# Amelie-Schreiber/ShapeMol

Measured on AMD Instinct MI355X. Metric: molecules/sec (1000-step DDPM sample, batch 256), higher is better.
Workload: dtype f32 (matrix operands split exactly into 3 x bf16 pieces = 24 bits, six piece products, fp32 accumulate); 1 GPU; BASELINE configs[1]: batch 256 MOSES-prior molecules (9-27 atoms) per GPU, 1000-step chain, fp32 results, k=8, synthetic shapes + hash-filled weights; besides the 5 warm-up steps an untimed 200-step chain runs first to reach the loaded clocks; batch_per_gpu=256, atoms_per_gpu=5541, total_atoms=5541, noise=device Philox, trajectories=kept in HBM, launch=hipGraph replay, parallelism=dp1 (whole batches per rank), ranks_seen=1

## Files before the change

### shapemol_amd/csrc/probe_node_only.hip

```cpp
#include "../../include/shapemol_hip.h"
#include "sm_device.h"
#include "sm_edge.h"
#include "sm_edge_bf16.h"
#include "sm_edge16.h"
#include "sm_node.h"
template __global__ void node_chain6_kernel<128>(NodeChainArgs);
template __global__ void node_linear6_kernel<128>(NodeLinArgs);
template __global__ void node_prologue6_kernel<128>(NodePrologueArgs);
```

### shapemol_amd/csrc/shapemol_hip.hip

```cpp
#include "../../include/shapemol_hip.h"
#include "sm_device.h"
#include "sm_edge.h"
#include "sm_edge_bf16.h"
#include "sm_edge16.h"
#include "sm_node.h"
#include "sm_node16.h"
#include "sm_edge_stream.h"
#include "sm_misc.h"
#include "sm_cfg.h"
#include "sm_guide_groups.h"
#include "sm_mesh.h"
#include <hip/hip_ext.h>

#include <algorithm>
#include <cmath>
#include <type_traits>
#include <cstdio>
#include <cstring>
#include <map>
#include <string>
#include <vector>

#include "sm_pack.h"

// ... 62 lines not shown
    float *x_a = nullptr, *x_b = nullptr, *x_state = nullptr, *pred_pos = nullptr, *pred_v = nullptr;
    int64_t *v_state = nullptr;
    unsigned long long *stamps = nullptr;
    unsigned long long *kstamps = nullptr;
    int kstamp_sel = -1;
    int stamp_on = 0;
    double *bn_acc = nullptr;
    int *status = nullptr;
    ChainParams *chain_params = nullptr;
    int64_t lastN = 0, lastB = 0;
    const float *last_h = nullptr, *last_x = nullptr;
    int stop_layer = -1, edge_threads = 0 , lin_waves = 16, edge_bf16 = 2, lin_bf16 = 1, chain_bf16 = 1, vn_fuse = 2;
    int vn_fold = 1;
    int max_mol_atoms = 0;
    int stream_whole_rounds = 0;
    int lin_fuse = 0;
    int bn_eval = 0;
    float *bn_run = nullptr;
    double *bn_eval_acc = nullptr;
    int ddpm_fold = 1;
    DdpmFold ddpm_vf{};
    int graph_fuse = 1;
    int x2h_chain = 1;
    int node_f16 = 0;
    int feat_f16 = 0;
    int edge_tiles = -1;
    float hid_max = 0.f;
    int num_cu = 256;
    CloudSet cs; MeshSet ms;
    int2 *wg_table = nullptr; int64_t wg_table_cap = 0;
    shapemol_sd_ctx *field_sd = nullptr; double field_lr = 0.0; int field_step = 0;
    float4 *m_within = nullptr; int *m_out = nullptr, *m_cnt = nullptr; int64_t m_cap = 0, m_cnt_cap = 0;
    int64_t m_flag_groups = 0;
    double cfg_w = 0.0, cfg_p = 0.0; int cfg_type = 0, cfg_has_bounds = 0; float cfg_lo[3] = {}, cfg_hi[3] = {};
    float *cfg_tr_pos_u = nullptr, *cfg_tr_v_u = nullptr;
    float *inv_u = nullptr, *add0_u = nullptr, *addp_u = nullptr, *ps_u = nullptr, *pred_pos_u = nullptr, *pred_v_u = nullptr;
    float *shape_zero = nullptr;
    ShapeTermArgs *prep_terms_u = nullptr; VnShapeArgs *prep_vn_u = nullptr;
    float *cfg_stat = nullptr; double *cfg_part = nullptr; unsigned *cfg_hist = nullptr;
    CfgGroupSet cgs;
    int *cfg_mol_grp = nullptr; int2 *cfg_blk_tab = nullptr; double *cfg_gpart = nullptr; int64_t cfg_tab_stride = 0;
    int first_step = 0;
    int *pin_off = nullptr, *pin_atom = nullptr, *pin_nbr = nullptr; int64_t n_pins = 0; int pin_steps = 0, pin_k = 0;
    bool prof_on = false;
    std::vector<ProfRec> prof;
    hipEvent_t cur_e0 = nullptr, cur_e1 = nullptr;
    hipGraphExec_t gexec = nullptr, gexec_u = nullptr;
    int64_t n_captures = 0;
    int64_t launch_rec[8] = {}, graph_rec[8] = {};
    struct GraphKey { int64_t N = 0, B = 0; Guide guide = Guide::None; int fold = 0, gfuse = 0;
                      int cfg = 0 ; double cfgv[9] = {};
                      int cfg_groups = 0;
                      uint64_t field_gen = 0; double field_lr = 0.0; int field_step = 0;
                      bool operator==(const GraphKey &o) const {
                          if (!(N == o.N && B == o.B && guide == o.guide && fold == o.fold && gfuse == o.gfuse && cfg == o.cfg &&
                                cfg_groups == o.cfg_groups && field_gen == o.field_gen && field_lr == o.field_lr &&
                                field_step == o.field_step)) return false;
                          for (int i = 0; i < 9; ++i) if (cfgv[i] != o.cfgv[i]) return false;
                          return true;
                      } } gkey{};
    hipStream_t gstream = nullptr; bool gstream_set = false;
    void drop_graphs() {
        if (!gexec && !gexec_u) return;
        if (!gstream_set || hipStreamSynchronize(gstream) != hipSuccess) hipDeviceSynchronize();
        if (gexec) { hipGraphExecDestroy(gexec); gexec = nullptr; }
        if (gexec_u) { hipGraphExecDestroy(gexec_u); gexec_u = nullptr; }
    }
    const float *P(size_t off) const { return d_img + off; }
};

namespace {

// ... 115 lines not shown
    constexpr int vn_tail = vn_red_doubles(12, H / 8) * 8 + 12 * 96 * 4;
    constexpr int fold = K <= 16 ? kVnFoldBytes : 0;
    constexpr int x16 = 2 * EdgeImage16<H, NT>::TOTAL * 4 + fold, h16 = (EdgeImage16<H, NT>::TOTAL + EdgeImage16<H, 1>::TOTAL) * 4 + vn_tail;
    ATTR(x16, edge16_kernel<H, K, false>); ATTR(x16, edge16_kernel<H, K, false, true>);
    ATTR(x16, edge16_loop_kernel<H, K, false>); ATTR(x16, edge16_loop_kernel<H, K, false, true>);
    ATTR(h16, edge16_kernel<H, K, true>); ATTR(h16, edge16_kernel<H, K, true, true>);
    ATTR(h16, edge16_loop_kernel<H, K, true>); ATTR(h16, edge16_loop_kernel<H, K, true, true>);
    ATTR((StreamMap<H, false>::O_TAIL * 4 + kVnFoldBytes), edge_stream_kernel<H, K, false>);
    ATTR((StreamMap<H, true>::O_TAIL * 4 + (NT + kStreamProducers) * 64 * 2 * 8), edge_stream_kernel<H, K, true>);
    if constexpr (K <= 16) {
        constexpr int xph = EdgePhaseImage<H, NT>::TOTAL * 4, hph = (EdgePhaseImage<H, NT>::TOTAL + EdgePhaseImage<H, 1>::TOTAL) * 4 + vn_tail;
        ATTR(x16, x2h_chain16_kernel<H, K>); ATTR(x16, x2h_chain16_kernel<H, K, true>);
        ATTR((EdgeBlob<H, false>::TOTAL * 4), edge_attention_kernel<H, K, false>); ATTR((EdgeBlob<H, true>::TOTAL * 4), edge_attention_kernel<H, K, true>);
        ATTR(xph, edge_fused_kernel<H, K, false, false>); ATTR(xph, edge_fused_kernel<H, K, false, true>);
        ATTR(hph, edge_fused_kernel<H, K, true, false>); ATTR(hph, edge_fused_kernel<H, K, true, true>);
    }
    return 0;
}

template <int H>
int set_edge_attr(int KP) {
    constexpr size_t pro6 = 2 * Chain6Lds<H>::FRAG * 16 + Chain6Lds<H>::PRE * 4, pro16 = 2 * Chain16Lds<H>::FRAG * 16 + Chain16Lds<H>::PRE * 4;
    ATTR(pro6, node_prologue6_kernel<H>); ATTR(Chain6Lds<H>::BYTES, node_chain6_kernel<H>); ATTR(kLin6Chunk * 3 * H * 32, node_linear6_kernel<H>);
    ATTR(pro16, node_prologue16_kernel<H>); ATTR(Chain16Lds<H>::BYTES, node_chain16_kernel<H>); ATTR(kLin16Chunk * 2 * H * 32, node_linear16_kernel<H>);
    ATTR(pro16, node_prologue16_kernel<H, true>); ATTR(Chain16Lds<H>::BYTES, node_chain16_kernel<H, true>); ATTR(kLin16Chunk * 2 * H * 32, node_linear16_kernel<H, true>);
    return KP == 8 ? set_edge_attr_k<H, 8>() : (KP == 16 ? set_edge_attr_k<H, 16>() : set_edge_attr_k<H, 32>());
}
#undef ATTR

#define SM_ARGS(...) __VA_ARGS__
#define LAUNCH_KP(name, K, KERNEL, TAIL, ...) LAUNCH(name, SMK((KERNEL<H, K SM_ARGS TAIL>), __VA_ARGS__))
#define DISPATCH_KP16(name, KERNEL, TAIL, ...)                                                      \
    do { if (KP == 8) LAUNCH_KP(name, 8, KERNEL, TAIL, __VA_ARGS__); else LAUNCH_KP(name, 16, KERNEL, TAIL, __VA_ARGS__); } while (0)
#define DISPATCH_KP(name, KERNEL, TAIL, ...)                                                        \
    do { if (KP > 16) LAUNCH_KP(name, 32, KERNEL, TAIL, __VA_ARGS__); else DISPATCH_KP16(name, KERNEL, TAIL, __VA_ARGS__); } while (0)
#define DISPATCH_KP_F16(DISPATCH, name, KERNEL, TAIL, ...)                                          \
    do { if (c->feat_f16) DISPATCH(name, KERNEL, (SM_ARGS TAIL, true), __VA_ARGS__); else DISPATCH(name, KERNEL, TAIL, __VA_ARGS__); } while (0)

static int edge_waves_for(const shapemol_ctx *c, int njobs) {
    if (c->edge_threads > 0) return c->edge_threads / 64;
    return std::max(4, std::min(12, (njobs + c->num_cu - 1) / c->num_cu));
}

template <int H, bool H2X>
int launch_edge(shapemol_ctx *c, hipStream_t s, const EdgeArgs &a) {
    const int KP = c->KP;
// ... 129 lines not shown
template <int H>
int launch_linear(shapemol_ctx *c, hipStream_t s, const char *name, const float *in, const float *wimg, const float *wimg6, const float *wimg16, const float *add_mol,
                  int ld_add, float *out, int ld_out, int n_out_tiles, int n_atoms, unsigned long long *stamps) {
    const int nwave = c->lin_waves;
    const int n_ct = (n_atoms + 15) / 16, ogroups = (n_out_tiles + nwave - 1) / nwave;
    const int want_groups = std::max(1, c->num_cu / ogroups);
    const int tpg = std::max(1, (n_ct + want_groups - 1) / want_groups);
    const int agroups = (n_ct + tpg - 1) / tpg;
    const bool f16 = c->lin_bf16 && c->node_f16;
    NodeLinArgs a{in, f16 ? wimg16 : (c->lin_bf16 ? wimg6 : wimg), add_mol, c->mol_of, out, n_atoms, n_out_tiles, tpg, ld_add, ld_out, stamps, nwave};
    if (f16) {
        const size_t shm = (size_t)std::min(tpg, kLin16Chunk) * 2 * H * 32;
        if (c->feat_f16) LAUNCH(name, SMK((node_linear16_kernel<H, true>), dim3(ogroups * agroups), dim3(nwave * 64), shm, s, a, c->status + ST_RANGE));
        else LAUNCH(name, SMK(node_linear16_kernel<H>, dim3(ogroups * agroups), dim3(nwave * 64), shm, s, a, c->status + ST_RANGE));
    } else if (c->lin_bf16) {
        const size_t shm = (size_t)std::min(tpg, kLin6Chunk) * 3 * H * 32;
        LAUNCH(name, SMK(node_linear6_kernel<H>, dim3(ogroups * agroups), dim3(nwave * 64), shm, s, a));
    } else {
        LAUNCH(name, SMK(node_linear_kernel<H>, dim3(ogroups * agroups), dim3(nwave * 64), 0, s, a));
    }
    return 0;
}

NodeFollow follow_of(const shapemol_ctx *c, const DevMlpImg &m, int mode, float *out, int ld_out, int n_store) {
    NodeFollow f{};
    f.w1img = c->P(m.w1img); f.b1 = c->P(m.b1); f.ln_g = c->P(m.g); f.ln_b = c->P(m.be);
    f.w1img6 = c->P(c->node_f16 ? m.w1img16 : m.w1img6); f.w2img6 = c->P(c->node_f16 ? m.w2img16 : m.w2img6);
    f.w2img = c->P(m.w2img); f.b2 = c->P(m.b2); f.out = out; f.ld_out = ld_out; f.n_store = n_store; f.mode = mode; f.nt2 = m.nt2;
    return f;
}

__global__ void knn_pin_kernel(const int *off, int n_steps, const int *atom, const int *pnbr, int k, int kp, const int *step_cur, int n_atoms, int *nbr) {
    const int step = *step_cur;
    if (step < 0 || step >= n_steps) return;
    const int lo = off[step], hi = off[step + 1];
    for (int e = lo + blockIdx.x * blockDim.x + threadIdx.x; e < hi; e += gridDim.x * blockDim.x) {
        const int i = atom[e];
        if (i < 0 || i >= n_atoms) continue;
        for (int sl = 0; sl < kp; ++sl) nbr[(size_t)i * kp + sl] = sl < k ? pnbr[(size_t)e * k + sl] : -1;
    }
}

template <int H>
int run_prep_shape(shapemol_ctx *c, hipStream_t s, int64_t B, const float *d_shape);

void swap_uncond(shapemol_ctx *c) {
// ... 158 lines not shown
    const int L = g.num_layers, hd = g.n_heads, C = g.num_classes, D = g.time_emb_dim, KP = c->KP;
    const int n = (int)N;
    AtomEmbArgs ae{c->P(c->dm.embw), c->P(c->dm.embb), v_in, c->mol_of, c->ttab, c->t_mol, sampling ? c->steps : nullptr,
                   c->steps + 1, c->bn_acc, c->h_a, n, H, C, D, t_first, L * kBnReplicas * 2 * hd + L};
    const int nlay = c->stop_layer >= 0 ? std::min(c->stop_layer, L) : L;
    const bool fused_prologue = c->chain_bf16 && c->lin_bf16;
    if (fused_prologue && c->prologue_tab) {
        if (c->tab_key != prologue_tab_key(c)) return fail("run_score: the prologue tables are not built for this precision mode");
        PrologueTabArgs ta{c->etab, c->q_tab, c->pre_tab, c->tab_flag, v_in, c->mol_of, c->t_mol, ae.step_ptr, ae.step_cur, c->bn_acc,
                           c->add0, c->h_a, c->q_x, c->pre0, c->status + ST_RANGE, n, C, g.num_timesteps, t_first, ae.bn_acc_len};
        LAUNCH("node_prologue", SMK(node_prologue_tab_kernel<H>, dim3((unsigned)((N * 16 + kProTabThreads - 1) / kProTabThreads)), dim3(kProTabThreads), 0, s, ta));
    } else if (fused_prologue) {
        NodePrologueArgs pa = prologue_args<H>(c, v_in, c->mol_of, c->t_mol, c->add0, c->h_a, c->q_x, c->pre0, n);
        pa.step_ptr = ae.step_ptr; pa.step_cur = ae.step_cur; pa.bn_acc = c->bn_acc; pa.bn_acc_len = ae.bn_acc_len; pa.t_first = t_first;
        if (nlay == 0) pa.n_lin_tiles = 0;
        pa.stamps = c->kstamp_sel == 5 ? c->kstamps : nullptr;
        if (launch_prologue<H>(c, s, pa)) return 1;
    } else {
        LAUNCH("embed", SMK(atom_embed_kernel, dim3((N * H + 255) / 256), dim3(256), 0, s, ae));
    }
    const bool graph_fused = sampling && c->graph_fuse && c->max_mol_atoms > 0 && c->max_mol_atoms <= kGraphCap && KP <= 32 && c->n_pins == 0;
    int64_t (&rec)[8] = c->launch_rec;
    std::fill(rec, rec + 8, 0);
    rec[0] = sampling; rec[1] = graph_fused; rec[7] = c->num_cu;
    if (c->edge_bf16 == 2 && nlay > 0) { rec[5] = stream_chunk(c, n); rec[6] = (stream_jobs(c, n) + rec[5] - 1) / rec[5]; }
    if (reuse_graph) {
    } else if (graph_fused) {
        GraphArgs ga{x_in, c->mol_span, n, g.knn, KP, c->nbr, c->P(c->dm.ew.w1), c->P(c->dm.ew.b1), c->P(c->dm.ew.g), c->P(c->dm.ew.be),
                     c->P(c->dm.ew.w2), c->P(c->dm.ew.b2), c->ew, c->status + ST_SPAN, c->kstamp_sel == 4 ? c->kstamps : nullptr};
        const int apb = kGraphWaves * (KP >= 16 ? 1 : 16 / KP);
        DISPATCH_KP("graph", graph_kernel, (), dim3((n + apb - 1) / apb), dim3(kGraphWaves * 64), 0, s, ga);
    } else LAUNCH("knn", SMK(knn_kernel, dim3((N + 3) / 4), dim3(256), 0, s, x_in, c->mol_of, c->mol_off, n, g.knn, KP, c->nbr));
    if (sampling && c->n_pins > 0 && !reuse_graph)
        LAUNCH("knn", SMK(knn_pin_kernel, dim3(32), dim3(256), 0, s, c->pin_off, c->pin_steps, c->pin_atom, c->pin_nbr, c->pin_k, KP, c->steps + 1, n, c->nbr));
    EdgeWeightArgs ea{x_in, c->nbr, c->P(c->dm.ew.w1), c->P(c->dm.ew.b1), c->P(c->dm.ew.g), c->P(c->dm.ew.be),
                      c->P(c->dm.ew.w2), c->P(c->dm.ew.b2), c->ew, n * KP, KP};
    if (!graph_fused && !reuse_graph) {
        const int tiles = (n * KP + 15) / 16;
        LAUNCH("edge_weight", SMK(edge_weight_kernel<H>, dim3((tiles + 3) / 4), dim3(256), 0, s, ea));
    }
    const float *cur_x = x_in;
    float *cur_h = c->h_a;
    constexpr int NT = H / 16;
    bool v_done = false;
    if (nlay > 0 && !fused_prologue) {
        const DevLayer &D0 = c->dm.layer[0];
// ... 46 lines not shown
        } else {
            EdgeArgs e{c->P(Dl.blob_x2h), pre_x, c->q_x, cur_x, c->nbr, c->ew, c->att, n, ld_pre_x, stamps_x};
            if (launch_edge<H, false>(c, s, e)) return 1;
        }
        {
            float *dst = (last && out_h) ? out_h : (cur_h == c->h_a ? c->h_b : c->h_a);
            NodeChainArgs na{};
            na.att = c->att; na.h = cur_h; na.h_out = dst; na.n_atoms = n;
            na.stamps = (c->kstamp_sel == 3 && l == 0) ? c->kstamps : nullptr;
            na.w1img = c->P(Dl.no.w1img); na.b1 = c->P(Dl.no.b1); na.ln_g = c->P(Dl.no.g); na.ln_b = c->P(Dl.no.be);
            na.w2img = c->P(Dl.no.w2img); na.b2 = c->P(Dl.no.b2);
            na.w1img6 = c->P(c->node_f16 ? Dl.no.w1img16 : Dl.no.w1img6); na.w2img6 = c->P(c->node_f16 ? Dl.no.w2img16 : Dl.no.w2img6);
            na.f[0] = follow_of(c, Dl.q_h2x, NODE_LN_RELU, c->q_h, H, H);
            na.n_follow = 1;
            if (has_next) { na.f[1] = follow_of(c, c->dm.layer[l + 1].q_x2h, NODE_LN_RELU, c->q_x, H, H); na.n_follow = 2; }
            else if (out_v) { na.f[1] = follow_of(c, c->dm.vhead, NODE_SSP, out_v, C, C); na.n_follow = 2; v_done = true; }
            const int n_ct = (n + 15) / 16;
            const int lin_tiles = (has_next && l + 1 < L ? 8 : 4) * NT;
            const bool lin_fused = c->chain_bf16 && c->lin_bf16 && c->node_f16 && c->lin_fuse;
            if (lin_fused) {
                na.lin_img16 = c->P(Dl.lin16_img); na.add_mol = c->addp + (size_t)l * c->capB * 8 * H; na.mol_of = c->mol_of;
                na.pre_out = c->preAB; na.n_lin_tiles = lin_tiles; na.ld_add = 8 * H; na.ld_out = 8 * H;
            }
            if (xc_fused) { rec[4] = 1; if (launch_x2h_chain<H>(c, s, xea, na)) return 1; }
            else if (c->chain_bf16 && c->node_f16 && c->feat_f16) LAUNCH("node_chain", SMK((node_chain16_kernel<H, true>), dim3((n_ct + CHAIN_COLS - 1) / CHAIN_COLS), dim3(H * 4), Chain16Lds<H>::BYTES, s, na, c->status + ST_RANGE));
            else if (c->chain_bf16 && c->node_f16) LAUNCH("node_chain", SMK(node_chain16_kernel<H>, dim3((n_ct + CHAIN_COLS - 1) / CHAIN_COLS), dim3(H * 4), Chain16Lds<H>::BYTES, s, na, c->status + ST_RANGE));
            else if (c->chain_bf16) LAUNCH("node_chain", SMK(node_chain6_kernel<H>, dim3((n_ct + CHAIN_COLS - 1) / CHAIN_COLS), dim3(H * 4), Chain6Lds<H>::BYTES, s, na));
            else LAUNCH("node_chain", SMK(node_chain_kernel<H>, dim3((n_ct + CHAIN_COLS - 1) / CHAIN_COLS), dim3(H * 4), 0, s, na));
            cur_h = dst;
            if (!lin_fused && launch_linear<H>(c, s, "node_pre", cur_h, c->P(Dl.lin_img), c->P(Dl.lin6_img), c->P(Dl.lin16_img), c->addp + (size_t)l * c->capB * 8 * H, 8 * H,
                                 c->preAB, 8 * H, lin_tiles, n, (c->kstamp_sel == 0 && l == 0) ? c->kstamps : nullptr)) return 1;
        }
        float *x_next = (last && out_pos) ? out_pos : ((cur_x == c->x_a) ? c->x_b : c->x_a);
        bool vn_done = false, stats_done = false;
        unsigned long long *stamps_h = (c->kstamp_sel == 2 && l == 0) ? c->kstamps : nullptr;
        if ((f16 || stream) && c->vn_fuse != 1) {
            const H2xPlan plan = h2x_plan(c, l, fold, has_next, half_tiles, stat_acc, cur_x, x_next, out_pos);
            pending = plan.pending; stats_done = plan.stats_done; vn_done = plan.vn_done;
            if (plan.ddpm.enable) c->ddpm_vf = plan.ddpm;
            rec[2] |= plan.pending.enable; rec[3] |= plan.ddpm.enable;
            if (f16) {
                Edge16Args ea{};
                ea.image_k = c->P(Dl.i16_kh); ea.image_v = c->P(Dl.i16_vh);
                fill_edge(ea, c, c->preAB, 8 * H, c->q_h, cur_x, c->o3, n, half_tiles, stamps_h);
                ea.vn = plan.vn; ea.xsum = plan.xsum;
                if (launch_edge16<H, true>(c, s, ea)) return 1;
            } else {
                EdgeStreamArgs sa{};
                sa.part_k = c->P(Dl.st_kh); sa.part_v = c->P(Dl.st_vh);
                sa.w2k = reinterpret_cast<const unsigned *>(c->P(Dl.sw2_kh));
                fill_edge(sa, c, c->preAB, 8 * H, c->q_h, cur_x, c->o3, n, half_tiles, stamps_h);
                sa.vn = plan.vn; sa.xsum = plan.xsum;
                if (launch_stream<H, true>(c, s, sa)) return 1;
// ... 318 lines not shown
    else if (k == "edge_bf16") {
        if (value < 0 || value > 3) return fail("edge_bf16 must be 0 (fp32 MFMA), 1 (exactly split bf16, phase kernels), 2 (exactly split bf16, streaming kernels) or 3 (two-piece f16)");
        if (value != 3 && value != 2 && c->KP > 16) return fail("k > 16 runs on the streaming (edge_bf16 = 2) or the two-piece f16 (edge_bf16 = 3) edge kernels");
        if (value == 3 && c->hid_max > 6.0e4f) return fail("edge_bf16 = 3: the edge MLPs' LayerNorm outputs may exceed the fp16 range for these weights");
        c->edge_bf16 = (int)value;
    }
    else if (k == "edge_tiles") { if (value < -1 || value > 1) return fail("edge_tiles must be -1 (automatic), 0 (sliced one-job launches) or 1 (looping launch)"); c->edge_tiles = (int)value; }
    else if (k == "node_f16") c->node_f16 = value != 0;
    else if (k == "feat_f16") {
        if (value && (c->edge_bf16 != 3 || !c->node_f16)) return fail("feat_f16 = 1 needs the f16 kernels (edge_bf16 = 3, node_f16 = 1)");
        c->feat_f16 = value != 0;
    }
    else if (k == "lin_fuse") c->lin_fuse = value != 0;
    else if (k == "stream_whole_rounds") c->stream_whole_rounds = value != 0;
    else if (k == "x2h_chain") c->x2h_chain = value != 0;
    else if (k == "graph_fuse") c->graph_fuse = value != 0;
    else if (k == "bn_eval") c->bn_eval = value != 0;
    else if (k == "ddpm_fold") c->ddpm_fold = value != 0;
    else if (k == "vn_fold") c->vn_fold = value != 0;
    else if (k == "prologue_tab") c->prologue_tab = value != 0;
    else if (k == "lin_bf16") c->lin_bf16 = (int)value;
    else if (k == "chain_bf16") c->chain_bf16 = (int)value;
    else if (k == "vn_fuse") c->vn_fuse = (int)value;
    else if (k == "lin_waves") { if (value < 1 || value > 16) return fail("lin_waves must be 1..16"); c->lin_waves = (int)value; }
    else if (k == "stamps") c->stamp_on = (int)value;
    else if (k == "kstamp_sel") c->kstamp_sel = (int)value;
    else if (k == "edge_waves") { if (value < 0 || value > 12) return fail("edge_waves must be 0 (automatic) .. 12"); c->edge_threads = (int)value * 64; }
    else return fail("unknown option " + k);
    hipSetDevice(c->device);
    c->drop_graphs();
    return 0;
}

int64_t shapemol_debug_read(shapemol_ctx *c, const char *name, void *dst, size_t max_bytes) {
    if (!c || !name || !dst) { fail("shapemol_debug_read: null argument"); return -1; }
    const std::string k(name);
    const shapemol_config &g = c->cfg;
    const int64_t N = c->lastN;
    const void *src = nullptr; size_t bytes = 0;
    int64_t dims[8] = {N, c->lastB, c->KP, g.hidden_dim, g.n_heads, g.num_layers, c->capN, c->capB};
    if (k == "dims") { if (max_bytes < sizeof(dims)) return -1; std::memcpy(dst, dims, sizeof(dims)); return sizeof(dims); }
    if (k == "captures") { if (max_bytes < 8) return -1; std::memcpy(dst, &c->n_captures, 8); return 8; }
    if (k == "launch") { if (max_bytes < sizeof(c->launch_rec)) return -1; std::memcpy(dst, c->launch_rec, sizeof(c->launch_rec)); return sizeof(c->launch_rec); }
    if (k == "nbr") { src = c->nbr; bytes = N * c->KP * 4; }
    else if (k == "ew") { src = c->ew; bytes = N * c->KP * 4; }
    else if (k == "h") { src = c->last_h; bytes = N * g.hidden_dim * 4; }
    else if (k == "x") { src = c->last_x; bytes = N * 3 * 4; }
    else if (k == "h0") { src = c->h_a; bytes = N * g.hidden_dim * 4; }
    else if (k == "q_x") { src = c->q_x; bytes = N * g.hidden_dim * 4; }
    else if (k == "pre0") { src = c->pre0; bytes = N * 4 * g.hidden_dim * 4; }
    else if (k == "add0") { src = c->add0; bytes = (size_t)c->lastB * 4 * g.hidden_dim * 4; }
    else if (k == "pre") { src = c->preAB; bytes = N * 8 * g.hidden_dim * 4; }
    else if (k == "q") { src = c->q_h; bytes = N * g.hidden_dim * 4; }
    else if (k == "att") { src = c->att; bytes = N * g.hidden_dim * 4; }
    else if (k == "o3") { src = c->o3; bytes = N * 48 * 4; }
    else if (k == "stamps") { src = c->stamps; bytes = 2048 * 8; }
    else if (k == "kstamps") { src = c->kstamps; bytes = (size_t)8 * 16 * 4096 * 8; }
    else if (k == "vn_err") { src = c->status + ST_VN_BARRIER; bytes = 4; }
    else if (k == "mesh_group_flags") { src = c->m_cnt ? c->m_cnt + 4 * c->m_cnt_cap : nullptr; bytes = (size_t)c->m_flag_groups * 4; }
    else if (k == "cfg_stat") { src = c->cfg_stat; bytes = 2 * 4; }
    else if (k == "cfg_group_stat") { src = c->cgs.last_groups > 0 ? c->cgs.stat : nullptr; bytes = (size_t)c->cgs.last_groups * 2 * 4; }
    else if (k == "bnstat") { src = c->bn_acc; bytes = (size_t)g.num_layers * kBnReplicas * 2 * g.n_heads * 8; }
    else { fail("shapemol_debug_read: unknown buffer " + k); return -1; }
    if (!src || bytes > max_bytes) { fail("shapemol_debug_read: buffer unavailable or destination too small"); return -1; }
    if (hipSetDevice(c->device) != hipSuccess || hipDeviceSynchronize() != hipSuccess ||
        hipMemcpy(dst, src, bytes, hipMemcpyDeviceToHost) != hipSuccess) { fail("shapemol_debug_read: copy failed"); return -1; }
// ... 163 lines not shown
```

### shapemol_amd/csrc/sm_node.h

```cpp
#pragma once
#include "sm_device.h"

enum NodeMode { NODE_LN_RELU = 1, NODE_SSP = 2 };
constexpr int kNodeThreads = 1024;

struct NodeLinArgs {
    const float *in;
    const float *wimg;
    const float *add_mol;
    const int *mol_of;
    float *out;
    int n_atoms, n_out_tiles, tiles_per_group;
    int ld_add, ld_out;
    unsigned long long *stamps;
    int nwave;
};

constexpr int kLinChunk = 8;

template <int H>
__global__ void __launch_bounds__(kNodeThreads)
node_linear_kernel(NodeLinArgs a) {
    constexpr int NT = H / 16;
    constexpr int XS = H + 16;
// ... 29 lines not shown
            if (a.add_mol && c + 1 < nc)
                add_nxt = ldg4(a.add_mol + (size_t)a.mol_of[min((cb + c + 1) * 16 + n, a.n_atoms - 1)] * a.ld_add + 16 * ot + 4 * g);
            const float *xrow = tiles + (c * 16 + n) * XS;
            f32x4 acc = {add_cur.x, add_cur.y, add_cur.z, add_cur.w};
#pragma unroll
            for (int t = 0; t < NT; ++t) {
                const float4 x = ldg4(xrow + 16 * t + 4 * g);
                acc = mfma16(w[t].x, x.x, acc);
                acc = mfma16(w[t].y, x.y, acc);
                acc = mfma16(w[t].z, x.z, acc);
                acc = mfma16(w[t].w, x.w, acc);
            }
            const int atom = (cb + c) * 16 + n;
            if (ot_ok && atom < a.n_atoms) stg4(a.out + (size_t)atom * a.ld_out + 16 * ot + 4 * g, float4{acc[0], acc[1], acc[2], acc[3]});
            add_cur = add_nxt;
        }
    }
    SM_STAMP(a.stamps, 2);
}

constexpr int kLin6Chunk = 8;

template <int H>
__global__ void __launch_bounds__(kNodeThreads)
node_linear6_kernel(NodeLinArgs a) {
    constexpr int NB = H / 32;
    extern __shared__ __attribute__((aligned(16))) unsigned char lin6_lds[];
    u32x4 *frag = reinterpret_cast<u32x4 *>(lin6_lds);
    const int lane = threadIdx.x & 63, wave = threadIdx.x >> 6;
    const int n = lane & 15, g = lane >> 4;
    const int nwave = a.nwave;
    const int ogroups = (a.n_out_tiles + nwave - 1) / nwave;
    const int ot_raw = (blockIdx.x % ogroups) * nwave + wave;
    const bool ot_ok = ot_raw < a.n_out_tiles;
    const int ot = ot_ok ? ot_raw : a.n_out_tiles - 1;
    const int ag = blockIdx.x / ogroups;
    const int n_ct = (a.n_atoms + 15) / 16;
    const int ct0 = ag * a.tiles_per_group, ct1 = min(ct0 + a.tiles_per_group, n_ct);

    u32x4 w[3][NB];
    {
        const u32x4 *wi = reinterpret_cast<const u32x4 *>(a.wimg) + (size_t)ot * 3 * NB * 64 + lane;
#pragma unroll
        for (int p = 0; p < 3; ++p)
#pragma unroll
            for (int b = 0; b < NB; ++b) w[p][b] = wi[(p * NB + b) * 64];
    }

    for (int cb = ct0; cb < ct1; cb += kLin6Chunk) {
        const int nc = min(kLin6Chunk, ct1 - cb);
        __syncthreads();
        for (int idx = threadIdx.x; idx < nc * NB * 64; idx += nwave * 64) {
            const int sl = idx & 63, sb = (idx >> 6) % NB, sc = idx / (64 * NB);
            const int at = min((cb + sc) * 16 + (sl & 15), a.n_atoms - 1);
            const float *src = a.in + (size_t)at * H + 32 * sb + 4 * (sl >> 4);
            const float4 v0 = ldg4(src), v1 = ldg4(src + 16);
            const float v[8] = {v0.x, v0.y, v0.z, v0.w, v1.x, v1.y, v1.z, v1.w};
            u32x4 hi, mid, lo;
            split3_bf16(v, hi, mid, lo);
            u32x4 *dst = frag + ((size_t)(sc * 3) * NB + sb) * 64 + sl;
            dst[0] = hi; dst[NB * 64] = mid; dst[2 * NB * 64] = lo;
        }
        __syncthreads();
        for (int c = 0; c < nc; c += 2) {
            const bool two = c + 1 < nc;
            const int atom0 = (cb + c) * 16 + n, atom1 = atom0 + 16;
            f32x4 acc0 = {0.f, 0.f, 0.f, 0.f}, acc1 = {0.f, 0.f, 0.f, 0.f};
            if (a.add_mol) {
                const float4 t0 = ldg4(a.add_mol + (size_t)a.mol_of[min(atom0, a.n_atoms - 1)] * a.ld_add + 16 * ot + 4 * g);
                const float4 t1 = ldg4(a.add_mol + (size_t)a.mol_of[min(atom1, a.n_atoms - 1)] * a.ld_add + 16 * ot + 4 * g);
                acc0 = f32x4{t0.x, t0.y, t0.z, t0.w}; acc1 = f32x4{t1.x, t1.y, t1.z, t1.w};
            }
            const u32x4 *f0 = frag + (size_t)(c * 3) * NB * 64 + lane;
            const u32x4 *f1 = frag + (size_t)((two ? c + 1 : c) * 3) * NB * 64 + lane;
#pragma unroll
            for (int b = 0; b < NB; ++b) {
                const u32x4 h0 = f0[b * 64], m0 = f0[(NB + b) * 64], l0 = f0[(2 * NB + b) * 64];
                const u32x4 h1 = f1[b * 64], m1 = f1[(NB + b) * 64], l1 = f1[(2 * NB + b) * 64];
                acc0 = mfma_bf16(w[2][b], h0, acc0); acc1 = mfma_bf16(w[2][b], h1, acc1);
                acc0 = mfma_bf16(w[1][b], m0, acc0); acc1 = mfma_bf16(w[1][b], m1, acc1);
                acc0 = mfma_bf16(w[0][b], l0, acc0); acc1 = mfma_bf16(w[0][b], l1, acc1);
                acc0 = mfma_bf16(w[1][b], h0, acc0); acc1 = mfma_bf16(w[1][b], h1, acc1);
                acc0 = mfma_bf16(w[0][b], m0, acc0); acc1 = mfma_bf16(w[0][b], m1, acc1);
                acc0 = mfma_bf16(w[0][b], h0, acc0); acc1 = mfma_bf16(w[0][b], h1, acc1);
            }
            if (ot_ok && atom0 < a.n_atoms) stg4(a.out + (size_t)atom0 * a.ld_out + 16 * ot + 4 * g, float4{acc0[0], acc0[1], acc0[2], acc0[3]});
            if (ot_ok && two && atom1 < a.n_atoms) stg4(a.out + (size_t)atom1 * a.ld_out + 16 * ot + 4 * g, float4{acc1[0], acc1[1], acc1[2], acc1[3]});
        }
    }
}

struct NodeMlpArgs {
    const float *in0;
    const float *in1;
    const float *w1img;
    const float *b1;
    const float *ln_g, *ln_b;
    const float *w2img;
    const float *b2;
    const float *resid;
    float *out;
    int ld_out, n_store, mode, nt2, n_atoms;
};

template <int H>
struct NodeMlpLds {
    static constexpr int NT = H / 16;
    static constexpr int TEAMS = (16 / NT) < 4 ? (16 / NT) : 4;
    static constexpr int XS = H + 16;
    static constexpr int TOTAL = TEAMS * 16 * XS;
};

// ... 633 lines not shown
        const float rstd = 1.0f / sqrtf(var + 1e-5f);
        const float4 g0 = ldg4(a.q.ln_g + fa), g1 = ldg4(a.q.ln_g + fa + 16), e0 = ldg4(a.q.ln_b + fa), e1 = ldg4(a.q.ln_b + fa + 16);
        const float ga[8] = {g0.x, g0.y, g0.z, g0.w, g1.x, g1.y, g1.z, g1.w};
        const float be[8] = {e0.x, e0.y, e0.z, e0.w, e1.x, e1.y, e1.z, e1.w};
#pragma unroll
        for (int i = 0; i < 8; ++i) v[i] = fmaxf((v[i] - mean) * rstd * ga[i] + be[i], 0.f);
        u32x4 hi, mid, lo;
        split3_bf16(v, hi, mid, lo);
        u32x4 *dst = fhid + (b * CC + (col >> 4)) * 64 + frag_slot(b, gg * 16 + (col & 15));
        dst[0] = hi; dst[NB * CC * 64] = mid; dst[2 * NB * CC * 64] = lo;
    }
    __syncthreads();
    if (onq) {
        const float4 b = ldg4(a.q.b2 + f0);
        f32x4 acc[CC];
#pragma unroll
        for (int c = 0; c < CC; ++c) acc[c] = f32x4{b.x, b.y, b.z, b.w};
        gemm6(wq1, fhid, acc);
#pragma unroll
        for (int c = 0; c < CC; ++c)
            if (atom_ok(c)) stg4(a.q.out + (size_t)atom_of(c) * a.q.ld_out + f0, float4{acc[c][0], acc[c][1], acc[c][2], acc[c][3]});
    }
}
```

Before: 376.1 molecules/s.

## Split node chain into output kernel plus merged follow-up/linear kernel

```diff
diff --git a/shapemol_amd/csrc/probe_node_only.hip b/shapemol_amd/csrc/probe_node_only.hip
--- a/shapemol_amd/csrc/probe_node_only.hip
+++ b/shapemol_amd/csrc/probe_node_only.hip
@@ -7,3 +7,5 @@
 template __global__ void node_chain6_kernel<128>(NodeChainArgs);
 template __global__ void node_linear6_kernel<128>(NodeLinArgs);
 template __global__ void node_prologue6_kernel<128>(NodePrologueArgs);
+template __global__ void node_out6_kernel<128>(NodeChainArgs);
+template __global__ void node_after6_kernel<128>(NodeAfterArgs);
diff --git a/shapemol_amd/csrc/shapemol_hip.hip b/shapemol_amd/csrc/shapemol_hip.hip
--- a/shapemol_amd/csrc/shapemol_hip.hip
+++ b/shapemol_amd/csrc/shapemol_hip.hip
@@ -108,6 +108,10 @@
     DdpmFold ddpm_vf{};
     int graph_fuse = 1;
     int x2h_chain = 1;
+    int node_levels = 1;
+    int after_order = 2;
+    int after_waves = 16;
+    int after_lin_wgs = 0;
     int node_f16 = 0;
     int feat_f16 = 0;
     int edge_tiles = -1;
@@ -134,6 +138,7 @@
     hipGraphExec_t gexec = nullptr, gexec_u = nullptr;
     int64_t n_captures = 0;
     int64_t launch_rec[8] = {}, graph_rec[8] = {};
+    int64_t node_rec[8] = {};
     struct GraphKey { int64_t N = 0, B = 0; Guide guide = Guide::None; int fold = 0, gfuse = 0;
                       int cfg = 0 ; double cfgv[9] = {};
                       int cfg_groups = 0;
@@ -295,6 +300,7 @@
 int set_edge_attr(int KP) {
     constexpr size_t pro6 = 2 * Chain6Lds<H>::FRAG * 16 + Chain6Lds<H>::PRE * 4, pro16 = 2 * Chain16Lds<H>::FRAG * 16 + Chain16Lds<H>::PRE * 4;
     ATTR(pro6, node_prologue6_kernel<H>); ATTR(Chain6Lds<H>::BYTES, node_chain6_kernel<H>); ATTR(kLin6Chunk * 3 * H * 32, node_linear6_kernel<H>);
+    ATTR(Out6Lds<H>::BYTES, node_out6_kernel<H>); ATTR(After6Lds<H>::bytes(kLin6Chunk), node_after6_kernel<H>);
     ATTR(pro16, node_prologue16_kernel<H>); ATTR(Chain16Lds<H>::BYTES, node_chain16_kernel<H>); ATTR(kLin16Chunk * 2 * H * 32, node_linear16_kernel<H>);
     ATTR(pro16, node_prologue16_kernel<H, true>); ATTR(Chain16Lds<H>::BYTES, node_chain16_kernel<H, true>); ATTR(kLin16Chunk * 2 * H * 32, node_linear16_kernel<H, true>);
     return KP == 8 ? set_edge_attr_k<H, 8>() : (KP == 16 ? set_edge_attr_k<H, 16>() : set_edge_attr_k<H, 32>());
@@ -470,6 +476,36 @@
     return 0;
 }
 
+constexpr int kAfterChunk = 6;
+template <int H>
+int launch_node_levels(shapemol_ctx *c, hipStream_t s, const NodeChainArgs &na, const float *lin_img6, const float *add_mol, int ld_add,
+                       float *out, int ld_out, int lin_tiles) {
+    constexpr int NT = H / 16;
+    const int n = na.n_atoms, n_ct = (n + 15) / 16, n_pairs = (n_ct + CHAIN_COLS - 1) / CHAIN_COLS;
+    LAUNCH("node_chain", SMK(node_out6_kernel<H>, dim3(n_pairs), dim3(H * 4), Out6Lds<H>::BYTES, s, na));
+    const int lw = c->after_waves, bw = std::max(lw, NT);
+    const int per_cu = bw <= 8 ? 2 : 1;
+    const int slots = c->num_cu * per_cu;
+    NodeAfterArgs a{};
+    a.f[0] = na.f[0]; a.f[1] = na.f[1];
+    a.n_pairs = n_pairs; a.n_fjobs = na.n_follow * n_pairs; a.order = c->after_order;
+    int tpg = 1;
+    if (lin_tiles > 0) {
+        const int ogroups = (lin_tiles + lw - 1) / lw;
+        const int lin_wgs = c->after_lin_wgs > 0 ? c->after_lin_wgs : std::max(slots - a.n_fjobs, slots / 2);
+        const int want_groups = std::max(1, lin_wgs / ogroups);
+        tpg = std::max(1, (n_ct + want_groups - 1) / want_groups);
+        a.n_ljobs = ogroups * ((n_ct + tpg - 1) / tpg);
+    }
+    a.lin_chunk = std::min(tpg, per_cu == 2 ? kAfterChunk : kLin6Chunk);
+    a.lin = NodeLinArgs{na.h_out, lin_img6, add_mol, c->mol_of, out, n, lin_tiles, tpg, ld_add, ld_out, nullptr, lw};
+    const size_t shm = After6Lds<H>::bytes(a.lin_chunk);
+    const int64_t rec[8] = {1, a.n_fjobs, a.n_ljobs, bw, a.order, tpg, a.lin_chunk, (int64_t)shm};
+    std::copy(rec, rec + 8, c->node_rec);
+    LAUNCH("node_pre", SMK(node_after6_kernel<H>, dim3(a.n_fjobs + a.n_ljobs), dim3(bw * 64), shm, s, a));
+    return 0;
+}
+
 NodeFollow follow_of(const shapemol_ctx *c, const DevMlpImg &m, int mode, float *out, int ld_out, int n_store) {
     NodeFollow f{};
     f.w1img = c->P(m.w1img); f.b1 = c->P(m.b1); f.ln_g = c->P(m.g); f.ln_b = c->P(m.be);
@@ -674,6 +710,7 @@
     const bool graph_fused = sampling && c->graph_fuse && c->max_mol_atoms > 0 && c->max_mol_atoms <= kGraphCap && KP <= 32 && c->n_pins == 0;
     int64_t (&rec)[8] = c->launch_rec;
     std::fill(rec, rec + 8, 0);
+    std::fill(c->node_rec, c->node_rec + 8, 0);
     rec[0] = sampling; rec[1] = graph_fused; rec[7] = c->num_cu;
     if (c->edge_bf16 == 2 && nlay > 0) { rec[5] = stream_chunk(c, n); rec[6] = (stream_jobs(c, n) + rec[5] - 1) / rec[5]; }
     if (reuse_graph) {
@@ -766,13 +803,16 @@
                 na.lin_img16 = c->P(Dl.lin16_img); na.add_mol = c->addp + (size_t)l * c->capB * 8 * H; na.mol_of = c->mol_of;
                 na.pre_out = c->preAB; na.n_lin_tiles = lin_tiles; na.ld_add = 8 * H; na.ld_out = 8 * H;
             }
-            if (xc_fused) { rec[4] = 1; if (launch_x2h_chain<H>(c, s, xea, na)) return 1; }
+            const bool levels = c->node_levels && c->chain_bf16 && c->lin_bf16 && !c->node_f16 && !lin_fused;
+            float *lin_add = c->addp + (size_t)l * c->capB * 8 * H;
+            if (levels) { if (launch_node_levels<H>(c, s, na, c->P(Dl.lin6_img), lin_add, 8 * H, c->preAB, 8 * H, lin_tiles)) return 1; }
+            else if (xc_fused) { rec[4] = 1; if (launch_x2h_chain<H>(c, s, xea, na)) return 1; }
             else if (c->chain_bf16 && c->node_f16 && c->feat_f16) LAUNCH("node_chain", SMK((node_chain16_kernel<H, true>), dim3((n_ct + CHAIN_COLS - 1) / CHAIN_COLS), dim3(H * 4), Chain16Lds<H>::BYTES, s, na, c->status + ST_RANGE));
             else if (c->chain_bf16 && c->node_f16) LAUNCH("node_chain", SMK(node_chain16_kernel<H>, dim3((n_ct + CHAIN_COLS - 1) / CHAIN_COLS), dim3(H * 4), Chain16Lds<H>::BYTES, s, na, c->status + ST_RANGE));
             else if (c->chain_bf16) LAUNCH("node_chain", SMK(node_chain6_kernel<H>, dim3((n_ct + CHAIN_COLS - 1) / CHAIN_COLS), dim3(H * 4), Chain6Lds<H>::BYTES, s, na));
             else LAUNCH("node_chain", SMK(node_chain_kernel<H>, dim3((n_ct + CHAIN_COLS - 1) / CHAIN_COLS), dim3(H * 4), 0, s, na));
             cur_h = dst;
-            if (!lin_fused && launch_linear<H>(c, s, "node_pre", cur_h, c->P(Dl.lin_img), c->P(Dl.lin6_img), c->P(Dl.lin16_img), c->addp + (size_t)l * c->capB * 8 * H, 8 * H,
+            if (!lin_fused && !levels && launch_linear<H>(c, s, "node_pre", cur_h, c->P(Dl.lin_img), c->P(Dl.lin6_img), c->P(Dl.lin16_img), lin_add, 8 * H,
                                  c->preAB, 8 * H, lin_tiles, n, (c->kstamp_sel == 0 && l == 0) ? c->kstamps : nullptr)) return 1;
         }
         float *x_next = (last && out_pos) ? out_pos : ((cur_x == c->x_a) ? c->x_b : c->x_a);
@@ -1137,6 +1177,10 @@
     else if (k == "lin_bf16") c->lin_bf16 = (int)value;
     else if (k == "chain_bf16") c->chain_bf16 = (int)value;
     else if (k == "vn_fuse") c->vn_fuse = (int)value;
+    else if (k == "node_levels") c->node_levels = value != 0;
+    else if (k == "after_order") { if (value < 0 || value > 2) return fail("after_order must be 0 (follow-up jobs first), 1 (interleaved) or 2 (linear jobs first)"); c->after_order = (int)value; }
+    else if (k == "after_waves") { if (value < 1 || value > 16) return fail("after_waves must be 1..16"); c->after_waves = (int)value; }
+    else if (k == "after_lin_wgs") { if (value < 0 || value > 4096) return fail("after_lin_wgs must be 0 (automatic) .. 4096"); c->after_lin_wgs = (int)value; }
     else if (k == "lin_waves") { if (value < 1 || value > 16) return fail("lin_waves must be 1..16"); c->lin_waves = (int)value; }
     else if (k == "stamps") c->stamp_on = (int)value;
     else if (k == "kstamp_sel") c->kstamp_sel = (int)value;
@@ -1157,6 +1201,7 @@
     if (k == "dims") { if (max_bytes < sizeof(dims)) return -1; std::memcpy(dst, dims, sizeof(dims)); return sizeof(dims); }
     if (k == "captures") { if (max_bytes < 8) return -1; std::memcpy(dst, &c->n_captures, 8); return 8; }
     if (k == "launch") { if (max_bytes < sizeof(c->launch_rec)) return -1; std::memcpy(dst, c->launch_rec, sizeof(c->launch_rec)); return sizeof(c->launch_rec); }
+    if (k == "launch_node") { if (max_bytes < sizeof(c->node_rec)) return -1; std::memcpy(dst, c->node_rec, sizeof(c->node_rec)); return sizeof(c->node_rec); }
     if (k == "nbr") { src = c->nbr; bytes = N * c->KP * 4; }
     else if (k == "ew") { src = c->ew; bytes = N * c->KP * 4; }
     else if (k == "h") { src = c->last_h; bytes = N * g.hidden_dim * 4; }
diff --git a/shapemol_amd/csrc/sm_node.h b/shapemol_amd/csrc/sm_node.h
--- a/shapemol_amd/csrc/sm_node.h
+++ b/shapemol_amd/csrc/sm_node.h
@@ -75,19 +75,16 @@
 constexpr int kLin6Chunk = 8;
 
 template <int H>
-__global__ void __launch_bounds__(kNodeThreads)
-node_linear6_kernel(NodeLinArgs a) {
+SM_DEV void linear6_job(const NodeLinArgs &a, int job, int chunk, u32x4 *frag) {
     constexpr int NB = H / 32;
-    extern __shared__ __attribute__((aligned(16))) unsigned char lin6_lds[];
-    u32x4 *frag = reinterpret_cast<u32x4 *>(lin6_lds);
     const int lane = threadIdx.x & 63, wave = threadIdx.x >> 6;
     const int n = lane & 15, g = lane >> 4;
     const int nwave = a.nwave;
     const int ogroups = (a.n_out_tiles + nwave - 1) / nwave;
-    const int ot_raw = (blockIdx.x % ogroups) * nwave + wave;
+    const int ot_raw = (job % ogroups) * nwave + wave;
     const bool ot_ok = ot_raw < a.n_out_tiles;
     const int ot = ot_ok ? ot_raw : a.n_out_tiles - 1;
-    const int ag = blockIdx.x / ogroups;
+    const int ag = job / ogroups;
     const int n_ct = (a.n_atoms + 15) / 16;
     const int ct0 = ag * a.tiles_per_group, ct1 = min(ct0 + a.tiles_per_group, n_ct);
 
@@ -100,8 +97,8 @@
             for (int b = 0; b < NB; ++b) w[p][b] = wi[(p * NB + b) * 64];
     }
 
-    for (int cb = ct0; cb < ct1; cb += kLin6Chunk) {
-        const int nc = min(kLin6Chunk, ct1 - cb);
+    for (int cb = ct0; cb < ct1; cb += chunk) {
+        const int nc = min(chunk, ct1 - cb);
         __syncthreads();
         for (int idx = threadIdx.x; idx < nc * NB * 64; idx += nwave * 64) {
             const int sl = idx & 63, sb = (idx >> 6) % NB, sc = idx / (64 * NB);
@@ -141,6 +138,13 @@
             if (ot_ok && two && atom1 < a.n_atoms) stg4(a.out + (size_t)atom1 * a.ld_out + 16 * ot + 4 * g, float4{acc1[0], acc1[1], acc1[2], acc1[3]});
         }
     }
+}
+
+template <int H>
+__global__ void __launch_bounds__(kNodeThreads)
+node_linear6_kernel(NodeLinArgs a) {
+    extern __shared__ __attribute__((aligned(16))) unsigned char lin6_lds[];
+    linear6_job<H>(a, blockIdx.x, kLin6Chunk, reinterpret_cast<u32x4 *>(lin6_lds));
 }
 
 struct NodeMlpArgs {
@@ -820,3 +824,241 @@
             if (atom_ok(c)) stg4(a.q.out + (size_t)atom_of(c) * a.q.ld_out + f0, float4{acc[c][0], acc[c][1], acc[c][2], acc[c][3]});
     }
 }
+
+template <int H>
+struct Team6 {
+    static constexpr int NT = H / 16, NB = H / 32, CC = CHAIN_COLS, XS = Chain6Lds<H>::XS;
+    static constexpr int LPC = NB * 4;
+    static_assert(CC == 2, "the normalise pass covers exactly 32 columns");
+    const int lane = threadIdx.x & 63, ot = threadIdx.x >> 6;
+    const int n = lane & 15, g = lane >> 4;
+    const int f0 = 16 * ot + 4 * g;
+
+    template <int KB>
+    SM_DEV void load_piece(const float *img, int p, u32x4 (&w)[3][KB]) const {
+        const u32x4 *wi = reinterpret_cast<const u32x4 *>(img) + (size_t)ot * 3 * KB * 64 + lane;
+#pragma unroll
+        for (int b = 0; b < KB; ++b) w[p][b] = wi[(p * KB + b) * 64];
+    }
+    template <int KB>
+    SM_DEV void load_w(const float *img, u32x4 (&w)[3][KB]) const {
+#pragma unroll
+        for (int p = 0; p < 3; ++p) load_piece(img, p, w);
+    }
+    template <int KB>
+    SM_DEV void gemm6(const u32x4 (&w)[3][KB], const u32x4 *f, f32x4 (&acc)[CC]) const {
+#pragma unroll
+        for (int b = 0; b < KB; ++b) {
+            u32x4 xh[CC], xm[CC], xl[CC];
+#pragma unroll
+            for (int c = 0; c < CC; ++c) {
+                xh[c] = f[((0 * KB + b) * CC + c) * 64 + frag_slot(b, lane)];
+                xm[c] = f[((1 * KB + b) * CC + c) * 64 + frag_slot(b, lane)];
+                xl[c] = f[((2 * KB + b) * CC + c) * 64 + frag_slot(b, lane)];
+            }
+#pragma unroll
+            for (int c = 0; c < CC; ++c) acc[c] = mfma_bf16(w[2][b], xh[c], acc[c]);
+#pragma unroll
+            for (int c = 0; c < CC; ++c) acc[c] = mfma_bf16(w[1][b], xm[c], acc[c]);
+#pragma unroll
+            for (int c = 0; c < CC; ++c) acc[c] = mfma_bf16(w[0][b], xl[c], acc[c]);
+#pragma unroll
+            for (int c = 0; c < CC; ++c) acc[c] = mfma_bf16(w[1][b], xh[c], acc[c]);
+#pragma unroll
+            for (int c = 0; c < CC; ++c) acc[c] = mfma_bf16(w[0][b], xm[c], acc[c]);
+#pragma unroll
+            for (int c = 0; c < CC; ++c) acc[c] = mfma_bf16(w[0][b], xh[c], acc[c]);
+        }
+    }
+    SM_DEV void store_pre(float *pre, const f32x4 (&acc)[CC]) const {
+#pragma unroll
+        for (int c = 0; c < CC; ++c) stg4(pre + (c * 16 + n) * XS + f0, float4{acc[c][0], acc[c][1], acc[c][2], acc[c][3]});
+    }
+    template <int KB>
+    SM_DEV void put_frag(u32x4 *fo, int sb, int sc, int sl, const float (&v)[8]) const {
+        u32x4 hi, mid, lo;
+        split3_bf16(v, hi, mid, lo);
+        u32x4 *dst = fo + (sb * CC + sc) * 64 + frag_slot(sb, sl);
+        dst[0] = hi; dst[KB * CC * 64] = mid; dst[2 * KB * CC * 64] = lo;
+    }
+    SM_DEV void normalise(const float *pre, int mode, const float *gam, const float *bet, u32x4 *fo) const {
+        const int col = ot * (64 / LPC) + lane / LPC, ln = lane % LPC;
+        const int b = ln >> 2, gg = ln & 3;
+        const int fa = 32 * b + 4 * gg;
+        const float4 p0 = ldg4(pre + col * XS + fa), p1 = ldg4(pre + col * XS + fa + 16);
+        float v[8] = {p0.x, p0.y, p0.z, p0.w, p1.x, p1.y, p1.z, p1.w};
+        if (mode == NODE_LN_RELU) {
+            float s = 0.f;
+#pragma unroll
+            for (int i = 0; i < 8; ++i) s += v[i];
+            const float mean = seg_sum<LPC>(s) * (1.0f / H);
+            float q = 0.f;
+#pragma unroll
+            for (int i = 0; i < 8; ++i) { const float d = v[i] - mean; q += d * d; }
+            const float var = seg_sum<LPC>(q) * (1.0f / H);
+            const float rstd = 1.0f / sqrtf(var + 1e-5f);
+            const float4 g0 = ldg4(gam + fa), g1 = ldg4(gam + fa + 16), b0 = ldg4(bet + fa), b1 = ldg4(bet + fa + 16);
+            const float ga[8] = {g0.x, g0.y, g0.z, g0.w, g1.x, g1.y, g1.z, g1.w};
+            const float be[8] = {b0.x, b0.y, b0.z, b0.w, b1.x, b1.y, b1.z, b1.w};
+#pragma unroll
+            for (int i = 0; i < 8; ++i) v[i] = fmaxf((v[i] - mean) * rstd * ga[i] + be[i], 0.f);
+        } else {
+#pragma unroll
+            for (int i = 0; i < 8; ++i) v[i] = (v[i] > 20.f ? v[i] : log1pf(expf(v[i]))) - 0.6931471805599453f;
+        }
+        put_frag<NB>(fo, b, col >> 4, gg * 16 + (col & 15), v);
+    }
+};
+
+template <int H>
+struct Out6Lds {
+    static constexpr size_t BYTES = (size_t)2 * Chain6Lds<H>::FRAG * 16 + (size_t)Chain6Lds<H>::PRE * 4;
+};
+
+template <int H>
+__global__ void __launch_bounds__(H * 4)
+node_out6_kernel(NodeChainArgs a) {
+    using L = Chain6Lds<H>;
+    constexpr int NT = H / 16, NB = H / 32, CC = CHAIN_COLS;
+    extern __shared__ __attribute__((aligned(16))) unsigned char out6_lds[];
+    u32x4 *fin = reinterpret_cast<u32x4 *>(out6_lds);
+    float *pre0 = reinterpret_cast<float *>(fin + 2 * L::FRAG);
+    const Team6<H> t;
+    const int ct0 = blockIdx.x * CC;
+    auto atom_of = [&](int c) { return min((ct0 + c) * 16 + t.n, a.n_atoms - 1); };
+    auto atom_ok = [&](int c) { return (ct0 + c) * 16 + t.n < a.n_atoms; };
+
+    u32x4 w1[3][2 * NB], w2[3][NB];
+    constexpr int SITER = CC * 2 * NB * 64 / (NT * 64);
+    float4 sv0[SITER], sv1[SITER];
+#pragma unroll
+    for (int it = 0; it < SITER; ++it) {
+        const int idx = threadIdx.x + it * NT * 64;
+        const int sl = idx & 63, sb = (idx >> 6) % (2 * NB), sc = idx / (64 * 2 * NB);
+        const int at = min((ct0 + sc) * 16 + (sl & 15), a.n_atoms - 1);
+        const float *src = (sb < NB ? a.att + (size_t)at * H + 32 * sb : a.h + (size_t)at * H + 32 * (sb - NB)) + 4 * (sl >> 4);
+        sv0[it] = ldg4(src); sv1[it] = ldg4(src + 16);
+    }
+    float4 hres[CC];
+#pragma unroll
+    for (int c = 0; c < CC; ++c) hres[c] = ldg4(a.h + (size_t)atom_of(c) * H + t.f0);
+    const float4 b1 = ldg4(a.b1 + t.f0), b2 = ldg4(a.b2 + t.f0);
+    t.load_w(a.w1img6, w1);
+#pragma unroll
+    for (int it = 0; it < SITER; ++it) {
+        const int idx = threadIdx.x + it * NT * 64;
+        const int sl = idx & 63, sb = (idx >> 6) % (2 * NB), sc = idx / (64 * 2 * NB);
+        const float v[8] = {sv0[it].x, sv0[it].y, sv0[it].z, sv0[it].w, sv1[it].x, sv1[it].y, sv1[it].z, sv1[it].w};
+        t.template put_frag<2 * NB>(fin, sb, sc, sl, v);
+    }
+    t.load_w(a.w2img6, w2);
+    __syncthreads();
+
+    {
+        f32x4 acc[CC];
+#pragma unroll
+        for (int c = 0; c < CC; ++c) acc[c] = f32x4{b1.x, b1.y, b1.z, b1.w};
+        t.gemm6(w1, fin, acc);
+        t.store_pre(pre0, acc);
+    }
+    __syncthreads();
+    t.normalise(pre0, NODE_LN_RELU, a.ln_g, a.ln_b, fin);
+    __syncthreads();
+    f32x4 acc[CC];
+#pragma unroll
+    for (int c = 0; c < CC; ++c) acc[c] = f32x4{b2.x, b2.y, b2.z, b2.w};
+    t.gemm6(w2, fin, acc);
+#pragma unroll
+    for (int c = 0; c < CC; ++c) {
+        const float4 hn = {acc[c][0] + hres[c].x, acc[c][1] + hres[c].y, acc[c][2] + hres[c].z, acc[c][3] + hres[c].w};
+        if (atom_ok(c)) stg4(a.h_out + (size_t)atom_of(c) * H + t.f0, hn);
+    }
+}
+
+struct NodeAfterArgs {
+    NodeLinArgs lin;
+    NodeFollow f[2];
+    int n_pairs;
+    int n_fjobs, n_ljobs;
+    int order;
+    int lin_chunk;
+};
+
+template <int H>
+struct After6Lds {
+    static constexpr size_t FOLLOW = (size_t)Chain6Lds<H>::FRAG * 16 + (size_t)Chain6Lds<H>::PRE * 4;
+    static constexpr size_t bytes(int lin_chunk) { const size_t l = (size_t)lin_chunk * 3 * H * 32; return l > FOLLOW ? l : FOLLOW; }
+};
+
+template <int H>
+__global__ void __launch_bounds__(kNodeThreads)
+node_after6_kernel(NodeAfterArgs a) {
+    using L = Chain6Lds<H>;
+    constexpr int NT = H / 16, NB = H / 32, CC = CHAIN_COLS;
+    extern __shared__ __attribute__((aligned(16))) unsigned char after6_lds[];
+    const int blk = blockIdx.x;
+    int fj = -1, lj = -1;
+    if (a.order == 0) { if (blk < a.n_fjobs) fj = blk; else lj = blk - a.n_fjobs; }
+    else if (a.order == 2) { if (blk < a.n_ljobs) lj = blk; else fj = blk - a.n_ljobs; }
+    else {
+        const long long tot = a.n_fjobs + a.n_ljobs;
+        const int lo = (int)((long long)blk * a.n_ljobs / tot), hi = (int)((long long)(blk + 1) * a.n_ljobs / tot);
+        if (hi > lo) lj = lo; else fj = blk - lo;
+    }
+    if (lj >= 0) {
+        if ((int)(threadIdx.x >> 6) >= a.lin.nwave) return;
+        linear6_job<H>(a.lin, lj, a.lin_chunk, reinterpret_cast<u32x4 *>(after6_lds));
+        return;
+    }
+    const Team6<H> t;
+    if (t.ot >= NT) return;
+    const NodeFollow &F = a.f[fj / a.n_pairs];
+    const int ct0 = (fj % a.n_pairs) * CC, n_atoms = a.lin.n_atoms;
+    u32x4 *fh = reinterpret_cast<u32x4 *>(after6_lds);
+    float *pre = reinterpret_cast<float *>(fh + L::FRAG);
+
+    static_assert(CC * NB * 64 == NT * 64, "one fragment per thread");
+    const int sl = t.lane, sb = t.ot % NB, sc = t.ot / NB;
+    const int at = min((ct0 + sc) * 16 + (sl & 15), n_atoms - 1);
+    const float *src = a.lin.in + (size_t)at * H + 32 * sb + 4 * (sl >> 4);
+    const float4 v0 = ldg4(src), v1 = ldg4(src + 16);
+    const float4 b1 = ldg4(F.b1 + t.f0);
+    u32x4 w1[3][NB], w2[3][NB];
+    t.load_w(F.w1img6, w1);
+    {
+        const float v[8] = {v0.x, v0.y, v0.z, v0.w, v1.x, v1.y, v1.z, v1.w};
+        t.template put_frag<NB>(fh, sb, sc, sl, v);
+    }
+    const bool on = t.ot < F.nt2;
+    if (on) { t.load_piece(F.w2img6, 2, w2); t.load_piece(F.w2img6, 1, w2); }
+    __syncthreads();
+    {
+        f32x4 acc[CC];
+#pragma unroll
+        for (int c = 0; c < CC; ++c) acc[c] = f32x4{b1.x, b1.y, b1.z, b1.w};
+        t.gemm6(w1, fh, acc);
+        t.store_pre(pre, acc);
+    }
+    if (on) t.load_piece(F.w2img6, 0, w2);
+    __syncthreads();
+    t.normalise(pre, F.mode, F.ln_g, F.ln_b, fh);
+    __syncthreads();
+    if (!on) return;
+    const float4 b = ldg4(F.b2 + t.f0);
+    f32x4 acc[CC];
+#pragma unroll
+    for (int c = 0; c < CC; ++c) acc[c] = f32x4{b.x, b.y, b.z, b.w};
+    t.gemm6(w2, fh, acc);
+#pragma unroll
+    for (int c = 0; c < CC; ++c) {
+        const int atom = (ct0 + c) * 16 + t.n;
+        if (atom >= n_atoms) continue;
+        if (t.f0 + 4 <= F.n_store && (F.ld_out & 3) == 0) {
+            stg4(F.out + (size_t)atom * F.ld_out + t.f0, float4{acc[c][0], acc[c][1], acc[c][2], acc[c][3]});
+        } else {
+#pragma unroll
+            for (int r = 0; r < 4; ++r)
+                if (t.f0 + r < F.n_store) F.out[(size_t)atom * F.ld_out + t.f0 + r] = acc[c][r];
+        }
+    }
+}
```

Result: faster. 388.3 molecules/s, median of 6 (+3.2%).
